# Tarekbouamer/Image-Retrieval-for-Image-Based-Localization

Hardware: AMD Instinct MI355X
Metric: images/sec extract + queries/sec 1M-desc kNN, ResNet50-GeM 1024×768 (higher is better)
Workload: dtype fp16

## Files before the change

image-retrieval-for-image-based-localization_amd/cirtorch/_engine.py:

```python

import contextlib
import ctypes
import os
import threading

import torch

PKG_DIR = os.path.dirname(os.path.dirname(os.path.abspath(__file__)))
LIB_PATH = os.environ.get("RR_LIB", os.path.join(PKG_DIR, "librr.so"))

RR_F32, RR_BF16, RR_F16, RR_I8 = 0, 1, 2, 3
RR_ACT_IDENTITY, RR_ACT_LEAKY = 0, 1
RR_POOL_GEM, RR_POOL_MAC, RR_POOL_SPOC = 0, 1, 2
RR_CONV_AFFINE, RR_CONV_RESIDUAL, RR_CONV_PERM32 = 1, 2, 4
RR_NHWC, RR_NCHW = 0, 1
RR_MATCH_NN, RR_MATCH_MNN, RR_MATCH_SNN, RR_MATCH_SMNN = 0, 1, 2, 3
RR_RESP_HARRIS, RR_RESP_GFTT, RR_RESP_HESSIAN, RR_RESP_DOG = 0, 1, 2, 3
RR_EPI_SAMPSON, RR_EPI_SYMMETRICAL = 0, 1
TUNE_KEYS = ("GEMM_CONFIG", "GEMM_STAGES", "GEMM_WIDE", "GEMM_ASTAT", "GEMM_XCD_MAP", "STREAM_1X1", "CONV3X3",
             "GRID_CUS", "GEMM8", "KNN_FUSED", "CONV3_PIPE", "STEM", "STREAM_XCD", "CONV3S", "WRES", "PAIR_MID",
             "WRES_RING")
globals().update(("RR_TUNE_" + name, key) for key, name in enumerate(TUNE_KEYS))
TUNE_SIZE_KEYS = {"PATCHNET_CHUNK": 32}
globals().update(("RR_TUNE_" + name, key) for name, key in TUNE_SIZE_KEYS.items())
RR_PATCHNET_HARDNET, RR_PATCHNET_SOSNET = 0, 1

_DTYPE_CODE = {torch.float32: RR_F32, torch.bfloat16: RR_BF16, torch.float16: RR_F16,
               torch.int8: RR_I8}


class ConvDesc(ctypes.Structure):
    _fields_ = [(n, ctypes.c_int) for n in ("n", "h", "w", "c_in", "ho", "wo", "c_out", "kh", "kw", "stride",
                                            "pad", "dil", "k_packed", "ldy", "act")] + \
               [("slope", ctypes.c_float), ("flags", ctypes.c_int)]


class Region(ctypes.Structure):
    _fields_ = [(n, ctypes.c_uint16) for n in ("y0", "x0", "h", "w")]


_vp, _i, _ll, _f, _d, _sz = ctypes.c_void_p, ctypes.c_int, ctypes.c_longlong, ctypes.c_float, ctypes.c_double, ctypes.c_size_t
_SIGS = {
    "rr_version": ([], _i),
    "rr_build_info": ([], ctypes.c_char_p),
    "rr_last_error": ([], ctypes.c_char_p),
    "rr_device_arch": ([ctypes.c_char_p, _i], _i),
    "rr_image_to_nhwc": ([_vp, _i, _i, _i, _i, ctypes.POINTER(_f), ctypes.POINTER(_f), _i, _vp, _i, _i, _vp], _i),
    "rr_conv2d_fused": ([_vp, _vp, _vp, _vp, _vp, _vp, ctypes.POINTER(ConvDesc), _i, _i, _vp], _i),
    "rr_conv1x1_pair": ([_vp, _ll, _i, _vp, _vp, _vp, _i, _vp, _vp, _vp, _vp, _vp, _i, _f, _vp, _vp, _vp, _i, _i, _f,
                         _vp, _vp, _i, _vp], _i),
    "rr_conv3x3_pair": ([_vp, _i, _i, _i, _vp, _vp, _vp, _i, _f, _vp, _vp, _vp, _i, _f, _vp, _vp, _vp, _vp, _vp, _vp, _vp, _vp, _i, _f,
                         _vp, _vp, _vp, _i, _i, _f, _vp, _vp, _vp, _i, _vp], _i),
    "rr_pack_conv_weights": ([_vp, _i, _i, _i, _i, _i, _i, _i, _vp, _i, _vp], _i),
    "rr_stem_pack_weights": ([_vp, _i, _i, _i, _i, _vp, _i, _vp], _i),
    "rr_stem_conv_pool": ([_vp, _i, _i, _i, ctypes.POINTER(_f), ctypes.POINTER(_f), _i, _vp, _vp, _vp, _i, _f, _vp,
                           _i, _i, _i, _vp], _i),
    "rr_stem_conv_pool_u8": ([_vp, _i, _i, _i, ctypes.POINTER(_f), ctypes.POINTER(_f), _i, _vp, _vp, _vp, _i, _f,
# ... 101 lines not shown
_lock = threading.Lock()


def lib():
    global _lib
    if _lib is None:
        with _lock:
            if _lib is None:
                if not os.path.exists(LIB_PATH):
                    raise RuntimeError("librr.so not found at %s — build it with "
                                       "`python -c 'import __graft_entry__ as g; g.build()'`" % LIB_PATH)
                handle = ctypes.CDLL(LIB_PATH)
                for name, (args, res) in _SIGS.items():
                    fn = getattr(handle, name)
                    fn.argtypes = args
                    fn.restype = res
                _lib = handle
    return _lib


def check(rc, what):
    if rc != 0:
        msg = lib().rr_last_error().decode(errors="replace")
        raise RuntimeError("%s failed (rc=%d): %s" % (what, rc, msg))


def _tune_key(name):
    name = str(name).upper()
    name = name[len("RR_TUNE_"):] if name.startswith("RR_TUNE_") else name
    if name in TUNE_KEYS:
        return TUNE_KEYS.index(name)
    if name in TUNE_SIZE_KEYS:
        return TUNE_SIZE_KEYS[name]
    try:
        return int(name)
    except ValueError:
        raise ValueError("unknown tuning key %r (one of %s, or a number)" % (name, ", ".join(TUNE_KEYS + tuple(TUNE_SIZE_KEYS))))


def get_tuning(key):
    value = ctypes.c_int()
    check(lib().rr_get_tuning(_tune_key(key), ctypes.byref(value)), "rr_get_tuning")
    return value.value


def set_tuning(key, value):
    check(lib().rr_set_tuning(_tune_key(key), int(value)), "rr_set_tuning")


@contextlib.contextmanager
def tuning(**values):
    saved = []
    try:
        for name, value in values.items():
            saved.append((name, get_tuning(name)))
            set_tuning(name, value)
        yield
    finally:
        for name, value in reversed(saved):
            set_tuning(name, value)


def apply_tuning_arg(arg):
    for kv in filter(None, (arg or "").split(",")):
        key, value = kv.split("=")
        set_tuning(key.strip(), int(value, 0))


def stream_ptr(device=None):
    return ctypes.c_void_p(torch.cuda.current_stream(device).cuda_stream)
# ... 27 lines not shown
```

image-retrieval-for-image-based-localization_amd/csrc/rr_c3pair.hip:

```cpp
#include "rr_internal.h"

#ifndef C3P_IG2
#define C3P_IG2 1
#endif

namespace rr {

namespace {

typedef __attribute__((ext_vector_type(4))) float cf32x4_t;
typedef __attribute__((ext_vector_type(4))) int ci32x4_t;

constexpr unsigned COOB = 0x80000000u;

__device__ __forceinline__ void cdma16(ci32x4_t rsrc, unsigned voff, unsigned lds_addr) {
    unsigned keep;
    lds_addr = __builtin_amdgcn_readfirstlane(lds_addr);
    asm volatile(
        "s_mov_b32 %0, m0\n\t"
        "s_mov_b32 m0, %3\n\t"
        "s_nop 0\n\t"
        "buffer_load_dwordx4 %1, %2, 0 offen lds\n\t"
        "s_mov_b32 m0, %0"
        : "=&s"(keep)
        : "v"(voff), "s"(rsrc), "s"(lds_addr)
        : "memory");
}

__device__ __forceinline__ ci32x4_t crsrc(const void* base, unsigned bytes) {
    const unsigned long long b = (unsigned long long)base;
    ci32x4_t r;
    r.x = __builtin_amdgcn_readfirstlane((int)(unsigned)b);
    r.y = __builtin_amdgcn_readfirstlane((int)((unsigned)(b >> 32) & 0xFFFFu));
    r.z = __builtin_amdgcn_readfirstlane((int)bytes);
    r.w = 0x00020000;
    int x = r.x, y = r.y, z = r.z;
    asm volatile("s_nop 4" : "+s"(x), "+s"(y), "+s"(z));
    r.x = x;
    r.y = y;
    r.z = z;
    return r;
}

__device__ __forceinline__ void cbar() { asm volatile("s_waitcnt lgkmcnt(0)\n\ts_barrier" ::: "memory"); }

template <int K>
__device__ __forceinline__ int cwswz(int row, int chunk) {
    const int f = K == 64 ? ((row >> 1) & 7) : (row & 15);
    return row * (K * 2) + ((chunk ^ f) << 4);
}

__device__ __forceinline__ void cpin(uint4& v) { asm volatile("" : "+v"(v.x), "+v"(v.y), "+v"(v.z), "+v"(v.w)); }

}

struct C3PairArgs {
    const bf16_t* t1;
    const bf16_t* w0;
    const float *s0, *h0;
    const bf16_t* w33;
    const float *s33, *h33;
    const bf16_t* w3;
    const float *s3, *h3;
    const bf16_t* res;
    const bf16_t* xp;
    const bf16_t* wp;
    const float *sp, *hp;
    const bf16_t* w1;
    const float *s1, *h1;
    bf16_t* y;
    bf16_t* z;
    int* queue;
    int n, h, w;
    int act2, act3, act1, act0;
    float slope2, slope3, slope1, slope0;
};

namespace {

template <int C1, bool PROJ, typename HT, bool CONV1 = false>
__global__ void __launch_bounds__(512, 1) k_c3pair(C3PairArgs a, int tiles_w, int tiles_hw, int ntiles) {
    static_assert(!CONV1 || PROJ, "conv1 in the launch: the stage's first block only");
    constexpr int TH = 4, TW = 32, TP = TH * TW, PITCH = 40;
    constexpr int NSLOT = (TH + 2) * PITCH, NP = NSLOT / 8;
    constexpr int PCW = TW + 2;
    constexpr int FN = 4;
    constexpr int K3 = 64, C3 = 256, NK3 = K3 / 32, NR3 = C3 / 32, NF1 = C1 / 16, NK1 = C3 / 32;
    static_assert(NSLOT % 8 == 0 && PITCH % 8 == 0, "row-invariant patch swizzle");
    __shared__ __attribute__((aligned(1024))) char sPatch[NSLOT * 128];
    __shared__ __attribute__((aligned(16))) char sT2[TP * 128];
    __shared__ __attribute__((aligned(16))) char sW3[C3 * K3 * 2];
    __shared__ __attribute__((aligned(16))) char sW1[C1 * C3 * 2];
    __shared__ __attribute__((aligned(16))) char sWp[PROJ ? C3 * K3 * 2 : 16];
    __shared__ __attribute__((aligned(16))) float sS3[C3], sH3[C3], sS1[C1], sH1[C1], sS2[64], sH2[64];
    __shared__ __attribute__((aligned(16))) float sSp[PROJ ? C3 : 4], sHp[PROJ ? C3 : 4];
    __shared__ __attribute__((aligned(16))) char sW0[CONV1 ? 64 * 64 * 2 : 16];
    __shared__ __attribute__((aligned(16))) float sS0[CONV1 ? 64 : 4], sH0[CONV1 ? 64 : 4];
    __shared__ int sTile[4];

    const int tid = threadIdx.x, lane = tid & 63;
    const int wave = __builtin_amdgcn_readfirstlane(tid >> 6);
    const bool role3 = wave < 4;
    const int r16 = lane & 15, kq = lane >> 4, lrow = lane >> 3, lch = lane & 7;
    const int H = a.h, W = a.w;

    for (int i = tid; i < C3 * K3 / 8; i += 512) {
        const int r = i / (K3 / 8), c = i - r * (K3 / 8);
        *reinterpret_cast<uint4*>(sW3 + cwswz<K3>(r, c)) = reinterpret_cast<const uint4*>(a.w3)[i];
        if constexpr (PROJ) *reinterpret_cast<uint4*>(sWp + cwswz<K3>(r, c)) = reinterpret_cast<const uint4*>(a.wp)[i];
    }
    for (int i = tid; i < C1 * C3 / 8; i += 512) {
        const int r = i / (C3 / 8), c = i - r * (C3 / 8);
        *reinterpret_cast<uint4*>(sW1 + cwswz<C3>(r, c)) = reinterpret_cast<const uint4*>(a.w1)[i];
    }
    for (int i = tid; i < C3; i += 512) {
        sS3[i] = a.s3[i];
        sH3[i] = a.h3[i];
        if constexpr (PROJ) {
            sSp[i] = a.sp[i];
            sHp[i] = a.hp[i];
        }
    }
    for (int i = tid; i < C1; i += 512) {
        sS1[i] = a.s1[i];
        sH1[i] = a.h1[i];
    }
    if (tid < 64) {
        sS2[tid] = a.s33[tid];
        sH2[tid] = a.h33[tid];
        if constexpr (CONV1) {
            sS0[tid] = a.s0[tid];
            sH0[tid] = a.h0[tid];
        }
    }
    if constexpr (CONV1)
        for (int i = tid; i < 64 * 64 / 8; i += 512) {
            const int r = i / 8, c = i - r * 8;
            *reinterpret_cast<uint4*>(sW0 + cwswz<64>(r, c)) = reinterpret_cast<const uint4*>(a.w0)[i];
        }
    const int wc = wave & 1, wpx = (wave >> 1) & 1;

    const int b = (int)blockIdx.x, G = (int)gridDim.x, xcd = b & 7;
    const int nt8 = ntiles >> 3, rt8 = ntiles & 7;
    const int s_x = xcd < rt8 ? xcd * (nt8 + 1) : rt8 * (nt8 + 1) + (xcd - rt8) * nt8;
    const int n_x = nt8 + (xcd < rt8 ? 1 : 0);
    auto fetch_tile = [&](int i) __attribute__((always_inline)) {
        if (a.queue) {
            const int v = atomicAdd(a.queue + xcd, 1);
            return v < n_x ? s_x + v : -1;
        }
        const int t = i * G + xcd * (G >> 3) + (b >> 3);
        return t < ntiles ? t : -1;
    };
    if (tid == 0) {
        sTile[0] = fetch_tile(0);
        sTile[1] = fetch_tile(1);
        sTile[2] = fetch_tile(2);
    }
    __syncthreads();
    auto tile_id = [&](int i) __attribute__((always_inline)) { return sTile[i & 3]; };
    if (tile_id(0) < 0) return;
    auto tile_org = [&](int t, int& img, int& oh0, int& ow0) __attribute__((always_inline)) {
        img = t / tiles_hw;
        const int rem = t - img * tiles_hw, th = rem / tiles_w;
        oh0 = th * TH;
        ow0 = (rem - th * tiles_w) * TW;
    };

    const ci32x4_t rsX = crsrc(a.t1, (unsigned)((long long)a.n * H * W * 64 * 2));
    const unsigned ldsP = (unsigned)(unsigned long long)sPatch;
    auto patch_dma = [&](int t, bool live) __attribute__((always_inline)) {
        int img = 0, oh0 = 0, ow0 = 0;
        if (live) tile_org(t, img, oh0, ow0);
        int lr = lrow;
        asm volatile("" : "+v"(lr));
#pragma unroll
        for (int u = 0; u < 8; ++u) {
            const int d = wave + 4 * u, q = d * 8 + lr;
            if (d >= NP) break;
            const int pr = q / PITCH, pc = q - pr * PITCH;
            const int hh = oh0 - 1 + pr, ww = ow0 - 1 + pc;
            unsigned off = COOB;
            if (live && pc < PCW && (unsigned)hh < (unsigned)H && (unsigned)ww < (unsigned)W)
                off = (unsigned)(((((long long)img * H + hh) * W + ww) * 64 + ((lch ^ lr) << 3)) * 2);
            cdma16(rsX, off, ldsP + d * 1024);
        }
    };
    h16_f32x4_t acc[2][FN];
    auto conv3x3 = [&](const uint4 (&areg)[2][18]) __attribute__((always_inline)) {
        int lc;
        asm volatile("v_mbcnt_lo_u32_b32 %0, -1, 0\n\tv_mbcnt_hi_u32_b32 %0, -1, %0" : "=v"(lc));
        lc &= 15;
        const char* base[FN][3][2];
#pragma unroll
        for (int j = 0; j < FN; ++j)
#pragma unroll
            for (int dx = 0; dx < 3; ++dx)
#pragma unroll
                for (int hs = 0; hs < 2; ++hs) {
                    const int q = (wpx * 2 + (j >> 1)) * PITCH + (j & 1) * 16 + lc + dx;
                    base[j][dx][hs] = sPatch + q * 128 + (((kq + 4 * hs) ^ (q & 7)) << 4);
                }
#pragma unroll
        for (int ii = 0; ii < 2; ++ii)
#pragma unroll
            for (int j = 0; j < FN; ++j) acc[ii][j] = (h16_f32x4_t){0.f, 0.f, 0.f, 0.f};
#pragma unroll
        for (int s = 0; s < 18; ++s) {
            const int tap = s >> 1, hs = s & 1, dy = tap / 3, dx = tap % 3;
            uint4 fb[FN];
#pragma unroll
            for (int j = 0; j < FN; ++j) fb[j] = *reinterpret_cast<const uint4*>(base[j][dx][hs] + dy * PITCH * 128);
#pragma unroll
            for (int ii = 0; ii < 2; ++ii)
#pragma unroll
                for (int j = 0; j < FN; ++j) acc[ii][j] = H16<HT>::mfma(areg[ii][s], fb[j], acc[ii][j]);
        }
    };
    auto convert_patch = [&](int t) __attribute__((always_inline)) {
        if constexpr (CONV1) {
            int img, oh0, ow0;
            tile_org(t, img, oh0, ow0);
            const bool leaky0 = a.act0 == RR_ACT_LEAKY;
            for (int f = wave; f < NP * 8 / 16; f += 4) {
                int q = f * 16 + r16;
                asm volatile("" : "+v"(q));
                const int pr = q / PITCH, pc = q - pr * PITCH;
                const int hh = oh0 - 1 + pr, ww = ow0 - 1 + pc;
                const bool valid = pc < PCW && (unsigned)hh < (unsigned)H && (unsigned)ww < (unsigned)W;
                char* slot = sPatch + q * 128;
                uint4 bx[2];
#pragma unroll
                for (int kk = 0; kk < 2; ++kk)
                    bx[kk] = *reinterpret_cast<const uint4*>(slot + (((4 * kk + kq) ^ (q & 7)) << 4));
                h16_f32x4_t c0[4];
#pragma unroll
                for (int ii = 0; ii < 4; ++ii) c0[ii] = (h16_f32x4_t){0.f, 0.f, 0.f, 0.f};
#pragma unroll
                for (int kk = 0; kk < 2; ++kk)
#pragma unroll
                    for (int ii = 0; ii < 4; ++ii) {
// ... 45 lines not shown
            }
            if (leaky2) {
#pragma unroll
                for (int r = 0; r < 8; ++r) v[r] = v[r] > 0.f ? v[r] : v[r] * a.slope2;
            }
            uint4 o;
            o.x = H16<HT>::pack2(v[0], v[1]);
            o.y = H16<HT>::pack2(v[2], v[3]);
            o.z = H16<HT>::pack2(v[4], v[5]);
            o.w = H16<HT>::pack2(v[6], v[7]);
            *reinterpret_cast<uint4*>(sT2 + p * 128 + (((4 * wc + kq) ^ (p & 7)) << 4)) = o;
        }
    };

    const int pw = wave - 4;
    const bool leaky3 = a.act3 == RR_ACT_LEAKY, leaky1 = a.act1 == RR_ACT_LEAKY;
    constexpr int NRQ = PROJ ? NK3 : NR3;
    auto strip_pixel = [&](int t, int k) __attribute__((always_inline)) {
        int img, oh0, ow0;
        tile_org(t, img, oh0, ow0);
        return ((long long)img * H + oh0 + (k >> 1)) * W + ow0 + (k & 1) * 16 + r16;
    };
    auto load_rq = [&](uint4 (&dst)[NRQ], long long p) __attribute__((always_inline)) {
        if constexpr (PROJ) {
            const bf16_t* ps = a.xp + p * K3 + 8 * kq;
#pragma unroll
            for (int kk = 0; kk < NK3; ++kk) dst[kk] = ld16_once(ps + kk * 32);
        } else {
            const bf16_t* rs = a.res + p * C3 + 8 * kq;
#pragma unroll
            for (int i2 = 0; i2 < NR3; ++i2) dst[i2] = ld16_once(rs + 32 * i2);
        }
    };
    auto pair_strip = [&](int k, long long p, const uint4 (&rv)[NRQ]) __attribute__((always_inline)) {
        uint4 bq[NK3];
        {
            const int q = k * 16 + r16;
#pragma unroll
            for (int kk = 0; kk < NK3; ++kk)
                bq[kk] = *reinterpret_cast<const uint4*>(sT2 + q * 128 + (((4 * kk + kq) ^ (q & 7)) << 4));
        }
        uint4 yq[NR3];
        constexpr int IG = C3P_IG2 ? 2 : 1;
#pragma unroll
        for (int i0 = 0; i0 < NR3; i0 += IG) {
            int abase = 0;
            asm volatile("" : "+v"(abase));
            h16_f32x4_t acc3[IG][2], pacc[IG][2];
#pragma unroll
            for (int g = 0; g < IG; ++g)
#pragma unroll
                for (int hh = 0; hh < 2; ++hh) acc3[g][hh] = pacc[g][hh] = (h16_f32x4_t){0.f, 0.f, 0.f, 0.f};
#pragma unroll
            for (int kk = 0; kk < NK3; ++kk)
#pragma unroll
                for (int g = 0; g < IG; ++g)
#pragma unroll
                    for (int hh = 0; hh < 2; ++hh) {
                        const uint4 av = *reinterpret_cast<const uint4*>(sW3 + abase + cwswz<K3>((2 * (i0 + g) + hh) * 16 + r16, kk * 4 + kq));
                        acc3[g][hh] = H16<HT>::mfma(av, bq[kk], acc3[g][hh]);
                    }
            if constexpr (PROJ) {
#pragma unroll
                for (int kk = 0; kk < NK3; ++kk)
#pragma unroll
                    for (int g = 0; g < IG; ++g)
#pragma unroll
                        for (int hh = 0; hh < 2; ++hh) {
                            const uint4 av = *reinterpret_cast<const uint4*>(sWp + abase + cwswz<K3>((2 * (i0 + g) + hh) * 16 + r16, kk * 4 + kq));
                            pacc[g][hh] = H16<HT>::mfma(av, rv[kk], pacc[g][hh]);
                        }
            }
#pragma unroll
            for (int g = 0; g < IG; ++g) {
                const int i2 = i0 + g;
                const int c = 32 * i2 + 8 * kq;
                float v[8];
#pragma unroll
                for (int r = 0; r < 4; ++r) {
                    v[r] = acc3[g][0][r] * sS3[c + r] + sH3[c + r];
                    v[4 + r] = acc3[g][1][r] * sS3[c + 4 + r] + sH3[c + 4 + r];
                }
                if constexpr (PROJ) {
#pragma unroll
                    for (int r = 0; r < 4; ++r) {
                        v[r] += pacc[g][0][r] * sSp[c + r] + sHp[c + r];
                        v[4 + r] += pacc[g][1][r] * sSp[c + 4 + r] + sHp[c + 4 + r];
                    }
                } else {
                    const uint4 qv = rv[i2];
                    const unsigned w4[4] = {qv.x, qv.y, qv.z, qv.w};
#pragma unroll
                    for (int r = 0; r < 4; ++r) {
                        v[2 * r] += H16<HT>::lo(w4[r]);
                        v[2 * r + 1] += H16<HT>::hi(w4[r]);
                    }
                }
                if (leaky3) {
#pragma unroll
                    for (int r = 0; r < 8; ++r) v[r] = v[r] > 0.f ? v[r] : v[r] * a.slope3;
                }
                yq[i2].x = H16<HT>::pack2(v[0], v[1]);
                yq[i2].y = H16<HT>::pack2(v[2], v[3]);
// ... 19 lines not shown
        for (int o2 = 0; o2 < NF1 / 2; ++o2) {
            const int c = 32 * o2 + 8 * kq;
            float v[8];
#pragma unroll
            for (int r = 0; r < 4; ++r) {
                v[r] = zacc[2 * o2][r] * sS1[c + r] + sH1[c + r];
                v[4 + r] = zacc[2 * o2 + 1][r] * sS1[c + 4 + r] + sH1[c + 4 + r];
            }
            if (leaky1) {
#pragma unroll
                for (int r = 0; r < 8; ++r) v[r] = v[r] > 0.f ? v[r] : v[r] * a.slope1;
            }
            uint4 o;
            o.x = H16<HT>::pack2(v[0], v[1]);
            o.y = H16<HT>::pack2(v[2], v[3]);
            o.z = H16<HT>::pack2(v[4], v[5]);
            o.w = H16<HT>::pack2(v[6], v[7]);
            st16_once(a.z + p * C1 + c, o);
        }
    };

    if (role3) {
        uint4 areg[2][18];
#pragma unroll
        for (int i = 0; i < 2; ++i)
#pragma unroll
            for (int ks = 0; ks < 18; ++ks)
                areg[i][ks] = *reinterpret_cast<const uint4*>(a.w33 + (long long)(32 * wc + 16 * i + r16) * 576 +
                                                              (ks >> 1) * 64 + 32 * (ks & 1) + 8 * kq);
#pragma unroll
        for (int i = 0; i < 2; ++i)
#pragma unroll
            for (int ks = 0; ks < 18; ++ks) cpin(areg[i][ks]);
        auto conv = [&]() __attribute__((always_inline)) { conv3x3(areg); };
        patch_dma(tile_id(0), true);
        asm volatile("s_waitcnt vmcnt(0)" ::: "memory");
        cbar();
        if constexpr (CONV1) {
            convert_patch(tile_id(0));
            cbar();
        }
        conv();
        if (wpx == 0) store_t2();
        cbar();
        patch_dma(tile_id(1), tile_id(1) >= 0);
        asm volatile("s_waitcnt vmcnt(0)" ::: "memory");
        cbar();
        for (int s = 0; tile_id(s) >= 0; ++s) {
            const bool more = tile_id(s + 1) >= 0;
            if (wpx == 1) store_t2();
            if constexpr (CONV1) {
                if (more) convert_patch(tile_id(s + 1));
                cbar();
            }
            if (more) conv();
            cbar();
            if (more) {
                if (wpx == 0) store_t2();
                const int t2i = tile_id(s + 2);
                patch_dma(t2i, t2i >= 0);
                if (tid == 0) sTile[(s + 3) & 3] = t2i >= 0 ? fetch_tile(s + 3) : -1;
                asm volatile("s_waitcnt vmcnt(0)" ::: "memory");
            }
            cbar();
        }
    } else {
        __builtin_amdgcn_s_setprio(1);
        uint4 rq[4][NRQ];
        load_rq(rq[0], strip_pixel(tile_id(0), pw));
        load_rq(rq[1], strip_pixel(tile_id(0), 4 + pw));
        cbar();
        if constexpr (CONV1) cbar();
        cbar();
        cbar();
        for (int s = 0; tile_id(s) >= 0; s += 2) {
            {
                const int t = tile_id(s);
                const bool n1 = tile_id(s + 1) >= 0;
                if (n1) load_rq(rq[2], strip_pixel(tile_id(s + 1), pw));
                if constexpr (CONV1) cbar();
                pair_strip(pw, strip_pixel(t, pw), rq[0]);
                cbar();
                if (n1) load_rq(rq[3], strip_pixel(tile_id(s + 1), 4 + pw));
                pair_strip(4 + pw, strip_pixel(t, 4 + pw), rq[1]);
                cbar();
            }
            if (tile_id(s + 1) >= 0) {
                const int t = tile_id(s + 1);
                const bool n2 = tile_id(s + 2) >= 0;
                if (n2) load_rq(rq[0], strip_pixel(tile_id(s + 2), pw));
                if constexpr (CONV1) cbar();
                pair_strip(pw, strip_pixel(t, pw), rq[2]);
                cbar();
                if (n2) load_rq(rq[1], strip_pixel(tile_id(s + 2), 4 + pw));
                pair_strip(4 + pw, strip_pixel(t, 4 + pw), rq[3]);
                cbar();
            }
        }
    }
}

// ... 15 lines not shown
        return fail(RR_EINVAL, "rr_conv3x3_pair: null pointer");
    const bool proj = residual == nullptr;
    if (proj && (!xp || !wp || !scalep || !shiftp))
        return fail(RR_EINVAL, "rr_conv3x3_pair: either residual or the projection (xp, wp, scalep, shiftp)");
    if (c_out != 64 && c_out != 128) return fail(RR_EINVAL, "rr_conv3x3_pair: c_out 64 or 128");
    if (proj && c_out != 64) return fail(RR_EINVAL, "rr_conv3x3_pair: the projection form takes c_out = 64");
    const bool conv1 = w0 != nullptr;
    if (conv1 && (!proj || !scale0 || !shift0 || ((uintptr_t)w0 & 15)))
        return fail(RR_EINVAL, "rr_conv3x3_pair: conv1 in the launch (w0) needs the projection form, scale0, shift0");
    if (conv1 && act0 != RR_ACT_IDENTITY && act0 != RR_ACT_LEAKY) return fail(RR_EINVAL, "rr_conv3x3_pair: act0");
    if (n <= 0 || h <= 0 || w <= 0 || h % 4 || w % 32) return fail(RR_EINVAL, "rr_conv3x3_pair: h % 4, w % 32");
    if ((long long)n * h * w * 64 * 2 >= (1ll << 31)) return fail(RR_EINVAL, "rr_conv3x3_pair: t1 over 2 GiB (split the batch)");
    for (const void* p : {t1, w33, w3, residual, xp, wp, w1, (const void*)y, (const void*)z})
        if ((uintptr_t)p & 15) return fail(RR_EINVAL, "rr_conv3x3_pair: 16-byte alignment required");
    if ((uintptr_t)tile_queue & 3) return fail(RR_EINVAL, "rr_conv3x3_pair: tile_queue alignment");
    for (int act : {act2, act3, act1})
        if (act != RR_ACT_IDENTITY && act != RR_ACT_LEAKY) return fail(RR_EINVAL, "rr_conv3x3_pair: activation");
    C3PairArgs a;
    a.t1 = (const bf16_t*)t1; a.w33 = (const bf16_t*)w33; a.s33 = scale2; a.h33 = shift2;
    a.w3 = (const bf16_t*)w3; a.s3 = scale3; a.h3 = shift3; a.res = (const bf16_t*)residual;
    a.xp = (const bf16_t*)xp; a.wp = (const bf16_t*)wp; a.sp = scalep; a.hp = shiftp;
    a.w1 = (const bf16_t*)w1; a.s1 = scale1; a.h1 = shift1; a.y = (bf16_t*)y; a.z = (bf16_t*)z;
    a.n = n; a.h = h; a.w = w; a.act2 = act2; a.act3 = act3; a.act1 = act1;
    a.slope2 = slope2; a.slope3 = slope3; a.slope1 = slope1; a.queue = tile_queue;
    a.w0 = (const bf16_t*)w0; a.s0 = scale0; a.h0 = shift0; a.act0 = act0; a.slope0 = slope0;
    const int tiles_w = w / 32, tiles_hw = (h / 4) * tiles_w;
    const long long ntl = (long long)n * tiles_hw;
    if (ntl >= (1ll << 31)) return fail(RR_EINVAL, "rr_conv3x3_pair: too many tiles");
    const int cus = grid_cus();
    int grid = (int)(ntl < cus ? ntl : cus) & ~7;
    if (grid < 8) grid = 8;
    const dim3 g((unsigned)grid), b(512);
    hipStream_t s = as_stream(stream);
    auto go = [&](auto hv) {
        using H = decltype(hv);
        if (conv1) hipLaunchKernelGGL((k_c3pair<64, true, H, true>), g, b, 0, s, a, tiles_w, tiles_hw, (int)ntl);
        else if (proj) hipLaunchKernelGGL((k_c3pair<64, true, H>), g, b, 0, s, a, tiles_w, tiles_hw, (int)ntl);
        else if (c_out == 64) hipLaunchKernelGGL((k_c3pair<64, false, H>), g, b, 0, s, a, tiles_w, tiles_hw, (int)ntl);
        else hipLaunchKernelGGL((k_c3pair<128, false, H>), g, b, 0, s, a, tiles_w, tiles_hw, (int)ntl);
    };
    if (dtype == RR_F16) go(f16_t{});
    else go(bf16_t{});
    return check_launch("rr_conv3x3_pair");
}
```

image-retrieval-for-image-based-localization_amd/csrc/rr_runtime.hip:

```cpp
#include "rr_internal.h"

#include <cstring>

namespace rr {

static thread_local std::string g_err;

static const char* tune_store(Tuning& t, int key, int v) {
    switch (key) {
        case RR_TUNE_GEMM_STAGES: v = v == 3 ? 3 : 2; break;
        case RR_TUNE_GEMM_WIDE:
        case RR_TUNE_GEMM_ASTAT:
        case RR_TUNE_GEMM_XCD_MAP: v = v != 0; break;
        case RR_TUNE_KNN_FUSED: v = v != 0 && !t.knn_fused_env_off; break;
        case RR_TUNE_GRID_CUS:
            if (v < 0) return "rr_set_tuning: RR_TUNE_GRID_CUS must be >= 0";
            break;
        case RR_TUNE_GEMM8: v = v < 0 ? 0 : ((v & 3) > 2 ? 2 : (v & 3)) | (v & Tuning::GEMM8_FLAGS); break;
        default: break;
    }
    t.*TUNE_KEYS[key].member = v;
    return nullptr;
}

// ... 344 lines not shown
static inline unsigned cast_blocks(long long n) {
    const long long b = (n + 1023) / 1024;
    return (unsigned)(b < (1ll << 20) ? (b > 0 ? b : 1) : (1ll << 20));
}

static inline unsigned nblk(long long total, int b) { return (unsigned)((total + b - 1) / b); }

}

using namespace rr;

extern "C" {

int rr_version(void) { return 1; }

const char* rr_last_error(void) { return g_err.c_str(); }

int rr_device_arch(char* buf, int buflen) {
    int dev = 0;
    if (hipGetDevice(&dev) != hipSuccess) return fail(RR_EHIP, "hipGetDevice failed");
    hipDeviceProp_t prop;
    if (hipGetDeviceProperties(&prop, dev) != hipSuccess) return fail(RR_EHIP, "hipGetDeviceProperties failed");
    std::strncpy(buf, prop.gcnArchName, buflen - 1);
    buf[buflen - 1] = 0;
    return RR_OK;
}

int rr_set_tuning(int key, int value) {
    if (key >= RR_TUNE_SIZE_BASE && key < RR_TUNE_SIZE_BASE + TUNE_NSIZEKEYS) {
        if (value < 1) return fail(RR_EINVAL, "rr_set_tuning: a size key must be >= 1");
        g_tune.*TUNE_SIZE_KEYS[key - RR_TUNE_SIZE_BASE].member = value;
        return RR_OK;
    }
    if (key < 0 || key >= TUNE_NKEYS) return fail(RR_EINVAL, "rr_set_tuning: unknown key");
    const char* err = tune_store(g_tune, key, value);
    return err ? fail(RR_EINVAL, err) : RR_OK;
}

int rr_get_tuning(int key, int* value) {
    if (key >= RR_TUNE_SIZE_BASE && key < RR_TUNE_SIZE_BASE + TUNE_NSIZEKEYS) {
        if (!value) return fail(RR_EINVAL, "rr_get_tuning: null value");
        *value = g_tune.*TUNE_SIZE_KEYS[key - RR_TUNE_SIZE_BASE].member;
        return RR_OK;
    }
    if (key < 0 || key >= TUNE_NKEYS) return fail(RR_EINVAL, "rr_get_tuning: unknown key");
    if (!value) return fail(RR_EINVAL, "rr_get_tuning: null value");
    *value = g_tune.*TUNE_KEYS[key].member;
    return RR_OK;
}

int rr_image_to_nhwc(const float* src, int n, int c, int h, int w, const float* mean_host,
                     const float* std_host, int do_normalize, void* dst, int c_pad, int dtype,
                     void* stream) {
    if (c > 4 || c_pad < c || n <= 0 || h <= 0 || w <= 0) return fail(RR_EINVAL, "rr_image_to_nhwc: bad shape");
    NormParams np{};
    for (int i = 0; i < c; ++i) {
        np.mean[i] = do_normalize ? mean_host[i] : 0.f;
        np.stdv[i] = do_normalize ? std_host[i] : 1.f;
    }
    long long total = (long long)n * h * w;
    if (dtype == RR_BF16 && c == 3 && c_pad == 8 && (((uintptr_t)dst) & 15) == 0)
        hipLaunchKernelGGL(k_image_to_nhwc_bf16x8, dim3(nblk(total, 256)), dim3(256), 0, as_stream(stream), src,
                           total, h * w, np, do_normalize, (uint4*)dst);
    else if (dtype == RR_BF16)
        hipLaunchKernelGGL(k_image_to_nhwc<bf16_t>, dim3(nblk(total, 256)), dim3(256), 0, as_stream(stream), src, n,
                           c, h * w, np, do_normalize, (bf16_t*)dst, c_pad);
    else if (dtype == RR_F16)
        hipLaunchKernelGGL(k_image_to_nhwc<f16_t>, dim3(nblk(total, 256)), dim3(256), 0, as_stream(stream), src, n,
                           c, h * w, np, do_normalize, (f16_t*)dst, c_pad);
    else if (dtype == RR_F32)
        hipLaunchKernelGGL(k_image_to_nhwc<float>, dim3(nblk(total, 256)), dim3(256), 0, as_stream(stream), src, n, c,
                           h * w, np, do_normalize, (float*)dst, c_pad);
    else
        return fail(RR_EINVAL, "rr_image_to_nhwc: dtype");
    return check_launch("rr_image_to_nhwc");
// ... 152 lines not shown
```

image-retrieval-for-image-based-localization_amd/csrc/rr_tuning.h:

```cpp
#pragma once

#include "../../include/rr.h"

namespace rr {

struct Tuning {
    int gemm_config = 0;
    int gemm_stages = 2;
    int gemm_wide = 1;
    int gemm_astat = 0;
    int gemm_xcd_map = 0;
    int stream_1x1 = 1;
    int conv3x3 = 1;
    int grid_cus = 0;
    int gemm8 = 1;
    int knn_fused = 1;
    int conv3_pipe = 1;
    int stem = 2;
    int stream_xcd = 1;
    int conv3s = 1;
    int wres = 2;
    int pair_mid = 1;
    int wres_ring = 1;
    int patchnet_chunk = 16384;
    bool knn_fused_env_off = false;

    static constexpr int GEMM8_FLAGS = 4 | 8 | 16 | 32 | 64 | 128 | 512;
    int gemm8_mode() const { return gemm8 & 3; }
    bool gemm8_tile() const { return gemm8 & 4; }
    bool gemm8h() const { return !(gemm8 & 8); }
    bool gemm8a() const { return !(gemm8 & 16); }
    bool gemm8s() const { return !(gemm8 & 32); }
    bool gemm8_pmajor() const { return !(gemm8 & 64); }
    bool gemm8a_tile() const { return gemm8 & 128; }
    bool gemm8_short_persist() const { return !(gemm8 & 512); }
};

extern Tuning g_tune;

struct TuneKey {
    int Tuning::*member;
    const char* env;
};

inline constexpr TuneKey TUNE_KEYS[] = {
    {&Tuning::gemm_config, nullptr},
    {&Tuning::gemm_stages, "RR_GEMM_STAGES"},
    {&Tuning::gemm_wide, "RR_GEMM_WIDE"},
    {&Tuning::gemm_astat, nullptr},
    {&Tuning::gemm_xcd_map, nullptr},
    {&Tuning::stream_1x1, nullptr},
    {&Tuning::conv3x3, nullptr},
    {&Tuning::grid_cus, nullptr},
    {&Tuning::gemm8, "RR_GEMM8"},
    {&Tuning::knn_fused, "RR_KNN_FUSED"},
    {&Tuning::conv3_pipe, nullptr},
    {&Tuning::stem, nullptr},
    {&Tuning::stream_xcd, nullptr},
    {&Tuning::conv3s, nullptr},
    {&Tuning::wres, nullptr},
    {&Tuning::pair_mid, nullptr},
    {&Tuning::wres_ring, nullptr},
};
constexpr int TUNE_NKEYS = sizeof(TUNE_KEYS) / sizeof(TUNE_KEYS[0]);
static_assert(TUNE_NKEYS == RR_TUNE_WRES_RING + 1, "one TUNE_KEYS row per rr_tune_key");

inline constexpr TuneKey TUNE_SIZE_KEYS[] = {
    {&Tuning::patchnet_chunk, nullptr},
};
constexpr int TUNE_NSIZEKEYS = sizeof(TUNE_SIZE_KEYS) / sizeof(TUNE_SIZE_KEYS[0]);
static_assert(TUNE_NSIZEKEYS == RR_TUNE_PATCHNET_CHUNK - RR_TUNE_SIZE_BASE + 1, "one TUNE_SIZE_KEYS row per rr_tune_size_key");

}
```

include/rr.h:

```cpp
#ifndef RR_H_
#define RR_H_

#include <stddef.h>
#include <stdint.h>

#ifdef __cplusplus
extern "C" {
#endif

enum rr_dtype { RR_F32 = 0, RR_BF16 = 1, RR_F16 = 2, RR_I8 = 3 };
enum rr_act { RR_ACT_IDENTITY = 0, RR_ACT_LEAKY = 1 };
enum rr_pool_mode { RR_POOL_GEM = 0, RR_POOL_MAC = 1, RR_POOL_SPOC = 2 };
enum rr_conv_flags { RR_CONV_AFFINE = 1, RR_CONV_RESIDUAL = 2, RR_CONV_PERM32 = 4 };
enum rr_layout { RR_NHWC = 0, RR_NCHW = 1 };

#define RR_OK 0
#define RR_EINVAL -1
#define RR_EHIP -2
#define RR_ENOSPACE -3

int rr_version(void);
const char* rr_build_info(void);
const char* rr_last_error(void);
int rr_device_arch(char* buf, int buflen);
// ... 222 lines not shown
int rr_describe_keypoints_pyramid(const void* x, int n, int c, int h, int w, int u8, const float* kpts, const int* count,
                                  int npts, double scale, const float* lafs, int orient, int orient_bins, int ps,
                                  int num_ang_bins, int num_spatial_bins, int rootsift, double clipval, float* desc,
                                  float* angles, float* lafs_out, void* workspace, size_t workspace_bytes, void* stream);

int rr_patch_affine_shape(const float* patches, long long B, int ps, double eps, float* out, void* stream);
int rr_ellipse_to_laf(const float* ells, long long B, float* lafs, void* stream);
size_t rr_laf_affine_shape_workspace_bytes(int n, int c, int h, int w, int npts, int ps);
int rr_laf_affine_shape(const void* x, int n, int c, int h, int w, int u8, const float* lafs, const int* count, int npts, int ps,
                        double eps, float* lafs_out, void* workspace, size_t workspace_bytes, void* stream);

#define RR_PATCHNET_HARDNET 0
#define RR_PATCHNET_SOSNET 1
size_t rr_patchnet_packed_bytes(void);
int rr_patchnet_pack(const float* const* weights, const float* const* means, const float* const* vars, void* packed,
                     size_t packed_bytes, void* stream);
size_t rr_patchnet_workspace_bytes(long long B);
int rr_patchnet_trunk(const float* patches, long long B, int variant, const void* packed, void* map, void* stream);
int rr_patchnet_head(const void* map, long long B, int variant, const void* packed, float* desc, void* stream);
int rr_patchnet_describe(const float* patches, long long B, int variant, const void* packed, float* desc, void* workspace,
                         size_t workspace_bytes, void* stream);

size_t rr_rank_workspace_bytes(long long n, int nq);
int rr_rank_full(const float* db_f32, long long n, const float* q_f32, int nq, int d, long long* out_idx,
                 void* workspace, size_t workspace_bytes, void* stream);

enum rr_tune_key { RR_TUNE_GEMM_CONFIG = 0, RR_TUNE_GEMM_STAGES = 1, RR_TUNE_GEMM_WIDE = 2,
                   RR_TUNE_GEMM_ASTAT = 3, RR_TUNE_GEMM_XCD_MAP = 4, RR_TUNE_STREAM_1X1 = 5,
                   RR_TUNE_CONV3X3 = 6, RR_TUNE_GRID_CUS = 7, RR_TUNE_GEMM8 = 8,
                   RR_TUNE_KNN_FUSED = 9, RR_TUNE_CONV3_PIPE = 10,
                   RR_TUNE_STEM = 11, RR_TUNE_STREAM_XCD = 12, RR_TUNE_CONV3S = 13,
                   RR_TUNE_WRES = 14, RR_TUNE_PAIR_MID = 15, RR_TUNE_WRES_RING = 16 };
enum rr_tune_size_key { RR_TUNE_SIZE_BASE = 32, RR_TUNE_PATCHNET_CHUNK = 32 };
int rr_set_tuning(int key, int value);
int rr_get_tuning(int key, int* value);

int rr_fill_unit_rows(float* out, long long rows, int d, unsigned long long seed,
                      long long row0, void* stream);
int rr_quantize_i8(const float* x, long long n, void* y, float* amax_dev, void* stream);
int rr_quantize_i8_rows(const float* x, int rows, int d, void* y, float* amax_rows, void* stream);
int rr_cast_f32_bf16(const float* x, void* y, long long n, void* stream);
int rr_cast_f32_f16(const float* x, void* y, long long n, void* stream);

#ifdef __cplusplus
}
#endif
#endif
```

Baseline: 5530.

## Double-buffer conv3x3 patch tiles and keep projection weights in registers in c3pair

New measurement: 5556 (median of 6 runs). No clear change (+0.5%).

```diff
diff --git a/image-retrieval-for-image-based-localization_amd/cirtorch/_engine.py b/image-retrieval-for-image-based-localization_amd/cirtorch/_engine.py
--- a/image-retrieval-for-image-based-localization_amd/cirtorch/_engine.py
+++ b/image-retrieval-for-image-based-localization_amd/cirtorch/_engine.py
@@ -23,6 +23,8 @@
 globals().update(("RR_TUNE_" + name, key) for key, name in enumerate(TUNE_KEYS))
 TUNE_SIZE_KEYS = {"PATCHNET_CHUNK": 32}
 globals().update(("RR_TUNE_" + name, key) for name, key in TUNE_SIZE_KEYS.items())
+TUNE_SCHED_KEYS = {"C3PAIR": 48}
+globals().update(("RR_TUNE_" + name, key) for name, key in TUNE_SCHED_KEYS.items())
 RR_PATCHNET_HARDNET, RR_PATCHNET_SOSNET = 0, 1
 
 _DTYPE_CODE = {torch.float32: RR_F32, torch.bfloat16: RR_BF16, torch.float16: RR_F16,
@@ -190,10 +192,12 @@
         return TUNE_KEYS.index(name)
     if name in TUNE_SIZE_KEYS:
         return TUNE_SIZE_KEYS[name]
+    if name in TUNE_SCHED_KEYS:
+        return TUNE_SCHED_KEYS[name]
     try:
         return int(name)
     except ValueError:
-        raise ValueError("unknown tuning key %r (one of %s, or a number)" % (name, ", ".join(TUNE_KEYS + tuple(TUNE_SIZE_KEYS))))
+        raise ValueError("unknown tuning key %r (one of %s, or a number)" % (name, ", ".join(TUNE_KEYS + tuple(TUNE_SIZE_KEYS) + tuple(TUNE_SCHED_KEYS))))
 
 
 def get_tuning(key):
diff --git a/image-retrieval-for-image-based-localization_amd/csrc/rr_c3pair.hip b/image-retrieval-for-image-based-localization_amd/csrc/rr_c3pair.hip
--- a/image-retrieval-for-image-based-localization_amd/csrc/rr_c3pair.hip
+++ b/image-retrieval-for-image-based-localization_amd/csrc/rr_c3pair.hip
@@ -2,6 +2,15 @@
 
 #ifndef C3P_IG2
 #define C3P_IG2 1
+#endif
+#ifndef C3P_PROBE
+#define C3P_PROBE 0
+#endif
+#ifndef C3P_WPR
+#define C3P_WPR 144
+#endif
+#ifndef C3P_SPLIT
+#define C3P_SPLIT 10
 #endif
 
 namespace rr {
@@ -51,6 +60,11 @@
 }
 
 __device__ __forceinline__ void cpin(uint4& v) { asm volatile("" : "+v"(v.x), "+v"(v.y), "+v"(v.z), "+v"(v.w)); }
+
+template <int V>
+struct CI {
+    static constexpr int value = V;
+};
 
 }
 
@@ -78,20 +92,25 @@
 
 namespace {
 
-template <int C1, bool PROJ, typename HT, bool CONV1 = false>
+template <int C1, bool PROJ, typename HT, bool CONV1 = false, bool DB = false>
 __global__ void __launch_bounds__(512, 1) k_c3pair(C3PairArgs a, int tiles_w, int tiles_hw, int ntiles) {
     static_assert(!CONV1 || PROJ, "conv1 in the launch: the stage's first block only");
+    static_assert(!DB || (C1 == 64 && !CONV1), "second patch buffer: it fits beside W1 of C1 = 64 only");
+    constexpr int SPLIT = C3P_SPLIT;
+    static_assert(SPLIT > 0 && SPLIT < 18, "both phases take K-steps");
+    constexpr int WPR = DB && PROJ ? C3P_WPR : 0, NWPV = WPR / 8;
+    static_assert(WPR % 16 == 0 && WPR <= 256, "whole 16-row fragments");
     constexpr int TH = 4, TW = 32, TP = TH * TW, PITCH = 40;
     constexpr int NSLOT = (TH + 2) * PITCH, NP = NSLOT / 8;
     constexpr int PCW = TW + 2;
     constexpr int FN = 4;
     constexpr int K3 = 64, C3 = 256, NK3 = K3 / 32, NR3 = C3 / 32, NF1 = C1 / 16, NK1 = C3 / 32;
     static_assert(NSLOT % 8 == 0 && PITCH % 8 == 0, "row-invariant patch swizzle");
-    __shared__ __attribute__((aligned(1024))) char sPatch[NSLOT * 128];
+    __shared__ __attribute__((aligned(1024))) char sPatch[(DB ? 2 : 1) * NSLOT * 128];
     __shared__ __attribute__((aligned(16))) char sT2[TP * 128];
     __shared__ __attribute__((aligned(16))) char sW3[C3 * K3 * 2];
     __shared__ __attribute__((aligned(16))) char sW1[C1 * C3 * 2];
-    __shared__ __attribute__((aligned(16))) char sWp[PROJ ? C3 * K3 * 2 : 16];
+    __shared__ __attribute__((aligned(16))) char sWp[PROJ ? (C3 - WPR) * K3 * 2 : 16];
     __shared__ __attribute__((aligned(16))) float sS3[C3], sH3[C3], sS1[C1], sH1[C1], sS2[64], sH2[64];
     __shared__ __attribute__((aligned(16))) float sSp[PROJ ? C3 : 4], sHp[PROJ ? C3 : 4];
     __shared__ __attribute__((aligned(16))) char sW0[CONV1 ? 64 * 64 * 2 : 16];
@@ -107,7 +126,8 @@
     for (int i = tid; i < C3 * K3 / 8; i += 512) {
         const int r = i / (K3 / 8), c = i - r * (K3 / 8);
         *reinterpret_cast<uint4*>(sW3 + cwswz<K3>(r, c)) = reinterpret_cast<const uint4*>(a.w3)[i];
-        if constexpr (PROJ) *reinterpret_cast<uint4*>(sWp + cwswz<K3>(r, c)) = reinterpret_cast<const uint4*>(a.wp)[i];
+        if constexpr (PROJ)
+            if (r >= WPR) *reinterpret_cast<uint4*>(sWp + cwswz<K3>(r - WPR, c)) = reinterpret_cast<const uint4*>(a.wp)[i];
     }
     for (int i = tid; i < C1 * C3 / 8; i += 512) {
         const int r = i / (C3 / 8), c = i - r * (C3 / 8);
@@ -169,7 +189,7 @@
 
     const ci32x4_t rsX = crsrc(a.t1, (unsigned)((long long)a.n * H * W * 64 * 2));
     const unsigned ldsP = (unsigned)(unsigned long long)sPatch;
-    auto patch_dma = [&](int t, bool live) __attribute__((always_inline)) {
+    auto patch_dma = [&](int t, bool live, int buf) __attribute__((always_inline)) {
         int img = 0, oh0 = 0, ow0 = 0;
         if (live) tile_org(t, img, oh0, ow0);
         int lr = lrow;
@@ -183,11 +203,12 @@
             unsigned off = COOB;
             if (live && pc < PCW && (unsigned)hh < (unsigned)H && (unsigned)ww < (unsigned)W)
                 off = (unsigned)(((((long long)img * H + hh) * W + ww) * 64 + ((lch ^ lr) << 3)) * 2);
-            cdma16(rsX, off, ldsP + d * 1024);
+            cdma16(rsX, off, ldsP + buf * (NSLOT * 128) + d * 1024);
         }
     };
     h16_f32x4_t acc[2][FN];
-    auto conv3x3 = [&](const uint4 (&areg)[2][18]) __attribute__((always_inline)) {
+    auto conv3x3 = [&](const uint4 (&areg)[2][18], auto s0c, auto s1c, int buf) __attribute__((always_inline)) {
+        constexpr int S0 = decltype(s0c)::value, S1 = decltype(s1c)::value;
         int lc;
         asm volatile("v_mbcnt_lo_u32_b32 %0, -1, 0\n\tv_mbcnt_hi_u32_b32 %0, -1, %0" : "=v"(lc));
         lc &= 15;
@@ -199,14 +220,17 @@
 #pragma unroll
                 for (int hs = 0; hs < 2; ++hs) {
                     const int q = (wpx * 2 + (j >> 1)) * PITCH + (j & 1) * 16 + lc + dx;
-                    base[j][dx][hs] = sPatch + q * 128 + (((kq + 4 * hs) ^ (q & 7)) << 4);
+                    base[j][dx][hs] = sPatch + buf * (NSLOT * 128) + q * 128 + (((kq + 4 * hs) ^ (q & 7)) << 4);
                 }
-#pragma unroll
-        for (int ii = 0; ii < 2; ++ii)
-#pragma unroll
-            for (int j = 0; j < FN; ++j) acc[ii][j] = (h16_f32x4_t){0.f, 0.f, 0.f, 0.f};
-#pragma unroll
-        for (int s = 0; s < 18; ++s) {
+        if constexpr (S0 == 0) {
+#pragma unroll
+            for (int ii = 0; ii < 2; ++ii)
+#pragma unroll
+                for (int j = 0; j < FN; ++j) acc[ii][j] = (h16_f32x4_t){0.f, 0.f, 0.f, 0.f};
+        }
+        if constexpr (C3P_PROBE == 2) return;
+#pragma unroll
+        for (int s = S0; s < S1; ++s) {
             const int tap = s >> 1, hs = s & 1, dy = tap / 3, dx = tap % 3;
             uint4 fb[FN];
 #pragma unroll
@@ -318,6 +342,7 @@
             for (int i2 = 0; i2 < NR3; ++i2) dst[i2] = ld16_once(rs + 32 * i2);
         }
     };
+    uint4 wpv[NWPV > 0 ? NWPV : 1];
     auto pair_strip = [&](int k, long long p, const uint4 (&rv)[NRQ]) __attribute__((always_inline)) {
         uint4 bq[NK3];
         {
@@ -325,6 +350,13 @@
 #pragma unroll
             for (int kk = 0; kk < NK3; ++kk)
                 bq[kk] = *reinterpret_cast<const uint4*>(sT2 + q * 128 + (((4 * kk + kq) ^ (q & 7)) << 4));
+        }
+        if constexpr (C3P_PROBE == 1) {
+#pragma unroll
+            for (int kk = 0; kk < NK3; ++kk) asm volatile("" ::"v"(bq[kk].x), "v"(bq[kk].y), "v"(bq[kk].z), "v"(bq[kk].w));
+#pragma unroll
+            for (int i = 0; i < NRQ; ++i) asm volatile("" ::"v"(rv[i].x), "v"(rv[i].y), "v"(rv[i].z), "v"(rv[i].w));
+            return;
         }
         uint4 yq[NR3];
         constexpr int IG = C3P_IG2 ? 2 : 1;
@@ -353,8 +385,13 @@
                     for (int g = 0; g < IG; ++g)
 #pragma unroll
                         for (int hh = 0; hh < 2; ++hh) {
-                            const uint4 av = *reinterpret_cast<const uint4*>(sWp + abase + cwswz<K3>((2 * (i0 + g) + hh) * 16 + r16, kk * 4 + kq));
-                            pacc[g][hh] = H16<HT>::mfma(av, rv[kk], pacc[g][hh]);
+                            const int rb = 2 * (i0 + g) + hh;
+                            if (rb * 16 < WPR) {
+                                pacc[g][hh] = H16<HT>::mfma(wpv[2 * rb + kk], rv[kk], pacc[g][hh]);
+                            } else {
+                                const uint4 av = *reinterpret_cast<const uint4*>(sWp + abase + cwswz<K3>(rb * 16 - WPR + r16, kk * 4 + kq));
+                                pacc[g][hh] = H16<HT>::mfma(av, rv[kk], pacc[g][hh]);
+                            }
                         }
             }
 #pragma unroll
@@ -440,8 +477,38 @@
         for (int i = 0; i < 2; ++i)
 #pragma unroll
             for (int ks = 0; ks < 18; ++ks) cpin(areg[i][ks]);
-        auto conv = [&]() __attribute__((always_inline)) { conv3x3(areg); };
-        patch_dma(tile_id(0), true);
+        auto conv = [&]() __attribute__((always_inline)) { conv3x3(areg, CI<0>{}, CI<18>{}, 0); };
+        if constexpr (DB) {
+            patch_dma(tile_id(0), true, 0);
+            asm volatile("s_waitcnt vmcnt(0)" ::: "memory");
+            cbar();
+            patch_dma(tile_id(1), tile_id(1) >= 0, 1);
+            conv();
+            if (wpx == 0) store_t2();
+            cbar();
+            asm volatile("s_waitcnt vmcnt(0)" ::: "memory");
+            cbar();
+            for (int s = 0; tile_id(s) >= 0; ++s) {
+                const bool more = tile_id(s + 1) >= 0;
+                const int nb = (s + 1) & 1;
+                if (wpx == 1) store_t2();
+                if (more) {
+                    const int t2i = tile_id(s + 2);
+                    patch_dma(t2i, t2i >= 0, nb ^ 1);
+                    conv3x3(areg, CI<0>{}, CI<SPLIT>{}, nb);
+                }
+                cbar();
+                if (more) {
+                    conv3x3(areg, CI<SPLIT>{}, CI<18>{}, nb);
+                    if (wpx == 0) store_t2();
+                    if (tid == 0) sTile[(s + 3) & 3] = tile_id(s + 2) >= 0 ? fetch_tile(s + 3) : -1;
+                    asm volatile("s_waitcnt vmcnt(0)" ::: "memory");
+                }
+                cbar();
+            }
+            return;
+        }
+        patch_dma(tile_id(0), true, 0);
         asm volatile("s_waitcnt vmcnt(0)" ::: "memory");
         cbar();
         if constexpr (CONV1) {
@@ -451,7 +518,7 @@
         conv();
         if (wpx == 0) store_t2();
         cbar();
-        patch_dma(tile_id(1), tile_id(1) >= 0);
+        patch_dma(tile_id(1), tile_id(1) >= 0, 0);
         asm volatile("s_waitcnt vmcnt(0)" ::: "memory");
         cbar();
         for (int s = 0; tile_id(s) >= 0; ++s) {
@@ -466,7 +533,7 @@
             if (more) {
                 if (wpx == 0) store_t2();
                 const int t2i = tile_id(s + 2);
-                patch_dma(t2i, t2i >= 0);
+                patch_dma(t2i, t2i >= 0, 0);
                 if (tid == 0) sTile[(s + 3) & 3] = t2i >= 0 ? fetch_tile(s + 3) : -1;
                 asm volatile("s_waitcnt vmcnt(0)" ::: "memory");
             }
@@ -475,6 +542,13 @@
     } else {
         __builtin_amdgcn_s_setprio(1);
         uint4 rq[4][NRQ];
+        if constexpr (NWPV > 0) {
+#pragma unroll
+            for (int f = 0; f < NWPV; ++f)
+                wpv[f] = reinterpret_cast<const uint4*>(a.wp)[((f >> 1) * 16 + r16) * (K3 / 8) + (f & 1) * 4 + kq];
+#pragma unroll
+            for (int f = 0; f < NWPV; ++f) cpin(wpv[f]);
+        }
         load_rq(rq[0], strip_pixel(tile_id(0), pw));
         load_rq(rq[1], strip_pixel(tile_id(0), 4 + pw));
         cbar();
@@ -556,10 +630,13 @@
     if (grid < 8) grid = 8;
     const dim3 g((unsigned)grid), b(512);
     hipStream_t s = as_stream(stream);
+    const bool db = g_tune.c3pair != 0 && !conv1 && c_out == 64;
     auto go = [&](auto hv) {
         using H = decltype(hv);
         if (conv1) hipLaunchKernelGGL((k_c3pair<64, true, H, true>), g, b, 0, s, a, tiles_w, tiles_hw, (int)ntl);
+        else if (proj && db) hipLaunchKernelGGL((k_c3pair<64, true, H, false, true>), g, b, 0, s, a, tiles_w, tiles_hw, (int)ntl);
         else if (proj) hipLaunchKernelGGL((k_c3pair<64, true, H>), g, b, 0, s, a, tiles_w, tiles_hw, (int)ntl);
+        else if (db) hipLaunchKernelGGL((k_c3pair<64, false, H, false, true>), g, b, 0, s, a, tiles_w, tiles_hw, (int)ntl);
         else if (c_out == 64) hipLaunchKernelGGL((k_c3pair<64, false, H>), g, b, 0, s, a, tiles_w, tiles_hw, (int)ntl);
         else hipLaunchKernelGGL((k_c3pair<128, false, H>), g, b, 0, s, a, tiles_w, tiles_hw, (int)ntl);
     };
diff --git a/image-retrieval-for-image-based-localization_amd/csrc/rr_runtime.hip b/image-retrieval-for-image-based-localization_amd/csrc/rr_runtime.hip
--- a/image-retrieval-for-image-based-localization_amd/csrc/rr_runtime.hip
+++ b/image-retrieval-for-image-based-localization_amd/csrc/rr_runtime.hip
@@ -400,6 +400,10 @@
         g_tune.*TUNE_SIZE_KEYS[key - RR_TUNE_SIZE_BASE].member = value;
         return RR_OK;
     }
+    if (key >= RR_TUNE_SCHED_BASE && key < RR_TUNE_SCHED_BASE + TUNE_NSCHEDKEYS) {
+        g_tune.*TUNE_SCHED_KEYS[key - RR_TUNE_SCHED_BASE].member = value != 0;
+        return RR_OK;
+    }
     if (key < 0 || key >= TUNE_NKEYS) return fail(RR_EINVAL, "rr_set_tuning: unknown key");
     const char* err = tune_store(g_tune, key, value);
     return err ? fail(RR_EINVAL, err) : RR_OK;
@@ -409,6 +413,11 @@
     if (key >= RR_TUNE_SIZE_BASE && key < RR_TUNE_SIZE_BASE + TUNE_NSIZEKEYS) {
         if (!value) return fail(RR_EINVAL, "rr_get_tuning: null value");
         *value = g_tune.*TUNE_SIZE_KEYS[key - RR_TUNE_SIZE_BASE].member;
+        return RR_OK;
+    }
+    if (key >= RR_TUNE_SCHED_BASE && key < RR_TUNE_SCHED_BASE + TUNE_NSCHEDKEYS) {
+        if (!value) return fail(RR_EINVAL, "rr_get_tuning: null value");
+        *value = g_tune.*TUNE_SCHED_KEYS[key - RR_TUNE_SCHED_BASE].member;
         return RR_OK;
     }
     if (key < 0 || key >= TUNE_NKEYS) return fail(RR_EINVAL, "rr_get_tuning: unknown key");
diff --git a/image-retrieval-for-image-based-localization_amd/csrc/rr_tuning.h b/image-retrieval-for-image-based-localization_amd/csrc/rr_tuning.h
--- a/image-retrieval-for-image-based-localization_amd/csrc/rr_tuning.h
+++ b/image-retrieval-for-image-based-localization_amd/csrc/rr_tuning.h
@@ -23,6 +23,7 @@
     int pair_mid = 1;
     int wres_ring = 1;
     int patchnet_chunk = 16384;
+    int c3pair = 1;
     bool knn_fused_env_off = false;
 
     static constexpr int GEMM8_FLAGS = 4 | 8 | 16 | 32 | 64 | 128 | 512;
@@ -71,4 +72,10 @@
 constexpr int TUNE_NSIZEKEYS = sizeof(TUNE_SIZE_KEYS) / sizeof(TUNE_SIZE_KEYS[0]);
 static_assert(TUNE_NSIZEKEYS == RR_TUNE_PATCHNET_CHUNK - RR_TUNE_SIZE_BASE + 1, "one TUNE_SIZE_KEYS row per rr_tune_size_key");
 
+inline constexpr TuneKey TUNE_SCHED_KEYS[] = {
+    {&Tuning::c3pair, nullptr},
+};
+constexpr int TUNE_NSCHEDKEYS = sizeof(TUNE_SCHED_KEYS) / sizeof(TUNE_SCHED_KEYS[0]);
+static_assert(TUNE_NSCHEDKEYS == RR_TUNE_C3PAIR - RR_TUNE_SCHED_BASE + 1, "one TUNE_SCHED_KEYS row per rr_tune_sched_key");
+
 }
diff --git a/include/rr.h b/include/rr.h
--- a/include/rr.h
+++ b/include/rr.h
@@ -278,6 +278,7 @@
                    RR_TUNE_STEM = 11, RR_TUNE_STREAM_XCD = 12, RR_TUNE_CONV3S = 13,
                    RR_TUNE_WRES = 14, RR_TUNE_PAIR_MID = 15, RR_TUNE_WRES_RING = 16 };
 enum rr_tune_size_key { RR_TUNE_SIZE_BASE = 32, RR_TUNE_PATCHNET_CHUNK = 32 };
+enum rr_tune_sched_key { RR_TUNE_SCHED_BASE = 48, RR_TUNE_C3PAIR = 48 };
 int rr_set_tuning(int key, int value);
 int rr_get_tuning(int key, int* value);
 
```
